# apple/ml-mdm

Measured on AMD Instinct MI355X. Metric: denoise-steps/sec, whole job = N x optimizer steps/s at per-GPU batch 64 (train fwd+bwd+optimizer, cc12m_64x64 U-Net), higher is better.
Workload: dtype bf16; 1 GPU; unet64 train step, per-GPU batch 64, global batch 64; global_batch=64, parallelism=dp1, settle_steps=15

## Files before the change

### ml-mdm_amd/csrc/gemm_conv.hip

```cpp
#include <stdio.h>
#include <stdlib.h>

#include <type_traits>
#include <utility>

#include "common.hpp"
#include "conv_args.hpp"

namespace mdm {



__device__ __forceinline__ void load4(const float* p, float (&o)[4]) {
  const f32x4 t = *reinterpret_cast<const f32x4*>(p);
  o[0] = t[0]; o[1] = t[1]; o[2] = t[2]; o[3] = t[3];
}
__device__ __forceinline__ void load4(const bf16* p, float (&o)[4]) {
  const bf16x4 t = *reinterpret_cast<const bf16x4*>(p);
  o[0] = (float)t[0]; o[1] = (float)t[1]; o[2] = (float)t[2]; o[3] = (float)t[3];
}

__device__ __attribute__((aligned(16))) uint4 g_zero_page[4] = {};


struct NoPrefetch { __device__ __forceinline__ void operator()() const {} };

template <typename T, int BM, int BN, int WM, int WN, int LDS_BYTES, typename AfterLds = NoPrefetch>
__device__ __forceinline__ void conv_epilogue(const ConvArgs& p, f32x4 (&acc)[BM / WM / 16][BN / WN / 16], char* smem,
                                              int m0, int n0, AfterLds after_lds = AfterLds()) {
  constexpr int EPV = Tr<T>::EPV;
  constexpr int NT_ = WM * WN * 64;
  constexpr int TM = BM / WM, TN = BN / WN;
  constexpr int MT = TM / 16, NT = TN / 16;
  const int tid = threadIdx.x, lane = tid & 63, wave = tid >> 6;
  const int wm = wave / WN, wn = wave % WN;
  const int quad = lane >> 4, l16 = lane & 15;
  T* __restrict__ Y = reinterpret_cast<T*>(p.y);
  T* __restrict__ Ypre = reinterpret_cast<T*>(p.ypre);
  const T* __restrict__ R = reinterpret_cast<const T*>(p.res);
  const T* __restrict__ AUX = reinterpret_cast<const T*>(p.aux);
  constexpr int OCH = BN / EPV;
  constexpr bool POW2 = (OCH & (OCH - 1)) == 0;
  constexpr int PITCH = BN * (int)sizeof(T) + (POW2 ? 0 : 16);
  constexpr int SWZ = POW2 ? (OCH >= 32 ? 32 : OCH) - 1 : 0;
  static_assert(BM * PITCH <= LDS_BYTES, "output tile must fit the k-loop LDS");
  if ((p.Cout % EPV) == 0) {
    f32x4 bv[NT];
#pragma unroll
    for (int j = 0; j < NT; ++j) {
      const int n = n0 + wn * TN + j * 16 + quad * 4;
      bv[j] = (p.bias && n < p.Cout) ? *reinterpret_cast<const f32x4*>(p.bias + n) : f32x4{0.f, 0.f, 0.f, 0.f};
    }
#pragma unroll
    for (int i = 0; i < MT; ++i) {
      const int ml = wm * TM + i * 16 + l16;
#pragma unroll
      for (int j = 0; j < NT; ++j) {
        const int nl = wn * TN + j * 16 + quad * 4;
        const f32x4 v = acc[i][j] + bv[j];
        constexpr int CPL = 16 / (4 * (int)sizeof(T));
        const int cl = nl / EPV;
        char* dst = smem + ml * PITCH + ((cl ^ (ml & SWZ)) << 4) + ((nl / 4) % CPL) * 8;
        if constexpr (sizeof(T) == 4) {
          *reinterpret_cast<f32x4*>(dst) = v;
        } else {
          *reinterpret_cast<bf16x4*>(dst) = bf16x4{(bf16)v[0], (bf16)v[1], (bf16)v[2], (bf16)v[3]};
        }
      }
    }
    constexpr int NCHP = BM * (BN / EPV) / NT_;
    constexpr bool AUX8 = sizeof(T) == 2 && kFfnAuxByte;
    const T* const PSRC = (p.act == 2 && AUX) ? AUX : R;
    uint4 pre[NCHP];
    if (AUX8 && p.act == 2 && AUX) {
      const unsigned char* const A8 = reinterpret_cast<const unsigned char*>(p.aux);
#pragma unroll
      for (int i = 0; i < NCHP; ++i) {
        const int idx = tid + i * NT_;
        const int row = idx / (BN / EPV), ch = idx - row * (BN / EPV);
        const int m = m0 + row, n = n0 + ch * EPV;
        pre[i] = uint4{0u, 0u, 0u, 0u};
        if (m < p.M && n < p.Cout) {
          const uint2 t = *reinterpret_cast<const uint2*>(A8 + (size_t)m * p.Cout + n);
          pre[i].x = t.x; pre[i].y = t.y;
        }
      }
    } else if (PSRC) {
#pragma unroll
      for (int i = 0; i < NCHP; ++i) {
        const int idx = tid + i * NT_;
        const int row = idx / (BN / EPV), ch = idx - row * (BN / EPV);
        const int m = m0 + row, n = n0 + ch * EPV;
        pre[i] = uint4{0u, 0u, 0u, 0u};
        if (m < p.M && n < p.Cout) {
          size_t o = (size_t)m * p.Cout + n;
          if (p.ps_cout > 0) {
            const int ph = n / p.ps_cout, co = n - ph * p.ps_cout;
            const int bw = m % p.ps_W, t_ = m / p.ps_W;
            const int bh = t_ % p.ps_H, img = t_ / p.ps_H;
            o = (((size_t)img * (2 * p.ps_H) + 2 * bh + (ph >> 1)) * (2 * p.ps_W) + 2 * bw + (ph & 1)) * p.ps_cout + co;
          }
          pre[i] = *reinterpret_cast<const uint4*>(PSRC + o);
        }
      }
    }
    __syncthreads();
    const int act = p.act;
    constexpr int NCH = BM * OCH / NT_;
    static_assert(NCH * NT_ == BM * OCH, "staged tile must divide evenly over the block");
    uint4 raw[NCH];
#pragma unroll
    for (int i = 0; i < NCH; ++i) {
      const int idx = tid + i * NT_;
      const int row = idx / OCH, ch = idx - row * OCH;
      raw[i] = *reinterpret_cast<const uint4*>(smem + row * PITCH + ((ch ^ (row & SWZ)) << 4));
    }
    __syncthreads();
    if (PSRC) __builtin_amdgcn_s_waitcnt(0x0F70);
    after_lds();
#pragma unroll
    for (int i = 0; i < NCH; ++i) {
      const int idx = tid + i * NT_;
      const int row = idx / OCH, ch = idx - row * OCH;
      const int m = m0 + row, n = n0 + ch * EPV;
      if (m >= p.M || n >= p.Cout) continue;
      size_t o = (size_t)m * p.Cout + n;
      if (p.ps_cout > 0) {
        const int ph = n / p.ps_cout, co = n - ph * p.ps_cout;
        const int bw = m % p.ps_W, t_ = m / p.ps_W;
        const int bh = t_ % p.ps_H, img = t_ / p.ps_H;
        o = (((size_t)img * (2 * p.ps_H) + 2 * bh + (ph >> 1)) * (2 * p.ps_W) + 2 * bw + (ph & 1)) * p.ps_cout + co;
      }
      if (act == 0 && !R) {
        *reinterpret_cast<uint4*>(Y + o) = raw[i];
        continue;
      }
      Chunk<T> c;
      c.load(reinterpret_cast<const T*>(&raw[i]));
      if (act == 1) {
        if (Ypre) {
          if constexpr (AUX8) {
            const uint2 code = {DGeluCode::enc4(&c.v[0]), DGeluCode::enc4(&c.v[4])};
            *reinterpret_cast<uint2*>(reinterpret_cast<unsigned char*>(p.ypre) + o) = code;
          } else {
            *reinterpret_cast<uint4*>(Ypre + o) = raw[i];
          }
        }
        gelu_vec<T, EPV>(c.v);
      } else if (act == 2) {
        if constexpr (AUX8) {
          float g[8];
          DGeluCode::dec4(pre[i].x, g);
          DGeluCode::dec4(pre[i].y, g + 4);
#pragma unroll
          for (int e = 0; e < EPV; ++e) c.v[e] *= g[e];
        } else {
          Chunk<T> ax;
          ax.load(reinterpret_cast<const T*>(&pre[i]));
          mul_dgelu_vec<T, EPV>(c.v, ax.v);
        }
      }
      if (R) {
        Chunk<T> rr;
        rr.load(reinterpret_cast<const T*>(&pre[i]));
#pragma unroll
        for (int e = 0; e < EPV; ++e) c.v[e] += rr.v[e];
      }
      c.store(Y + o);
    }
    return;
  }
  __syncthreads();
  after_lds();
#pragma unroll
  for (int i = 0; i < MT; ++i) {
    const int m = m0 + wm * TM + i * 16 + l16;
    if (m >= p.M) continue;
#pragma unroll
    for (int j = 0; j < NT; ++j) {
      const int n = n0 + wn * TN + j * 16 + quad * 4;
      if (n >= p.Cout) continue;
      float v[4] = {acc[i][j][0], acc[i][j][1], acc[i][j][2], acc[i][j][3]};
      const size_t o = (size_t)m * p.Cout + n;
      const int nv = min(4, p.Cout - n);
#pragma unroll
      for (int e = 0; e < 4; ++e) {
        if (e >= nv) continue;
        if (p.bias) v[e] += p.bias[n + e];
        if (p.act == 1) {
          if (Ypre) {
            if constexpr (sizeof(T) == 2 && kFfnAuxByte) reinterpret_cast<unsigned char*>(p.ypre)[o + e] = (unsigned char)DGeluCode::enc(to_f32(from_f32<T>(v[e])));
            else Ypre[o + e] = from_f32<T>(v[e]);
          }
          v[e] = gelu_t<T>(v[e]);
        } else if (p.act == 2) {
          if constexpr (sizeof(T) == 2 && kFfnAuxByte) v[e] *= DGeluCode::dec(reinterpret_cast<const unsigned char*>(p.aux)[o + e]);
          else v[e] *= dgelu_t<T>(to_f32(AUX[o + e]));
        }
        if (R) v[e] += to_f32(R[o + e]);
        Y[o + e] = from_f32<T>(v[e]);
      }
    }
  }
}

__device__ __forceinline__ void load_frag_planes(FragSplit& f, const char* t, int row, int quad) {
  f.hi = *reinterpret_cast<const bf16x8*>(t + lds_chunk_off(row, 2 * quad));
  f.lo = *reinterpret_cast<const bf16x8*>(t + lds_chunk_off(row, 2 * quad + 1));
}
template <typename F> __device__ __forceinline__ void load_frag_planes(F&, const char*, int, int) {}

template <typename T, int BM, int BN, int WM, int WN, int MODE, int SPLIT = 0>
__global__ __launch_bounds__(WM * WN * 64, 2) void conv_gemm_kernel(ConvArgs p) {
  constexpr int NSTAGE = 2;
  constexpr int EPV = Tr<T>::EPV, BK = Tr<T>::BK, KSTEPS = Tr<T>::KSTEPS;
  constexpr int NT_ = WM * WN * 64;
  constexpr int RPP = NT_ / 8;
  constexpr int TM = BM / WM, TN = BN / WN;
  constexpr int MT = TM / 16, NT = TN / 16;
  constexpr int AJ = BM / RPP, BJ = BN / RPP;
  constexpr int A_BYTES = BM * 128, B_BYTES = BN * 128, STAGE = A_BYTES + B_BYTES;
  static_assert(BM % RPP == 0 && BN % RPP == 0, "tile rows must be a multiple of the staging pass");
  extern __shared__ __attribute__((aligned(16))) char smem[];

  const int tid = threadIdx.x, lane = tid & 63, wave = tid >> 6;
  const int wm = wave / WN, wn = wave % WN;
  const int quad = lane >> 4, l16 = lane & 15;

  const int tiles_n = (p.Cout + BN - 1) / BN;
  const int t = xcd_remap(blockIdx.x, gridDim.x);
  const int m0 = (t / tiles_n) * BM, n0 = (t % tiles_n) * BN;

  const T* __restrict__ X = reinterpret_cast<const T*>(p.x);
  const T* __restrict__ Wp = reinterpret_cast<const T*>(p.w);

  const int lrow = tid >> 3;
  const int lchunk = (tid & 7) ^ (lrow & 7);
  int a_pix[AJ];
  int a_oh[AJ], a_ow[AJ];
#pragma unroll
  for (int j = 0; j < AJ; ++j) {
    const int m = m0 + lrow + RPP * j;
    if (m < p.M) {
      if (MODE == MODE_1x1) {
        a_pix[j] = m; a_oh[j] = 0; a_ow[j] = 0;
      } else {
        const int hw = p.Ho * p.Wo;
        const int n = m / hw, r = m - n * hw;
        const int oh = r / p.Wo;
        a_pix[j] = n * p.H * p.W; a_oh[j] = oh; a_ow[j] = r - oh * p.Wo;
      }
    } else {
      a_pix[j] = -1; a_oh[j] = 0; a_ow[j] = 0;
    }
  }
  int kcur = lchunk * EPV;
// ... 47 lines not shown

  f32x4 acc[MT][NT];
#pragma unroll
  for (int i = 0; i < MT; ++i)
#pragma unroll
    for (int j = 0; j < NT; ++j) acc[i][j] = f32x4{0.f, 0.f, 0.f, 0.f};

  const int ntiles = (p.K + BK - 1) / BK;
#define MDM_COMPUTE_TILE(cur)                                                                             \
  {                                                                                                       \
    const char* As = (cur);                                                                               \
    const char* Bs = (cur) + A_BYTES;                                                                     \
    _Pragma("unroll") for (int ks = 0; ks < KSTEPS; ++ks) {                                               \
      typename FragOf<T, SPLIT != 0>::type af[MT], bfr[NT];                                               \
      _Pragma("unroll") for (int i = 0; i < MT; ++i) load_frag_x(af[i], As, wm * TM + i * 16 + l16, ks, quad);    \
      _Pragma("unroll") for (int j = 0; j < NT; ++j) {                                                    \
        if constexpr (SPLIT == 2) load_frag_planes(bfr[j], Bs, wn * TN + j * 16 + l16, quad);             \
        else load_frag_x(bfr[j], Bs, wn * TN + j * 16 + l16, ks, quad);                                   \
      }                                                                                                   \
      _Pragma("unroll") for (int i = 0; i < MT; ++i)                                                      \
        _Pragma("unroll") for (int j = 0; j < NT; ++j) mma16(acc[i][j], bfr[j], af[i]);                   \
    }                                                                                                     \
  }
  MDM_STAGE_TILE(smem);
  __syncthreads();
  for (int kt = 0; kt < ntiles; ++kt) {
    char* cur = smem + (kt & 1) * STAGE;
    if (kt + 1 < ntiles) MDM_STAGE_TILE(smem + ((kt + 1) & 1) * STAGE);
    MDM_COMPUTE_TILE(cur);
    __syncthreads();
  }
#undef MDM_COMPUTE_TILE
#undef MDM_STAGE_TILE
#undef MDM_GLDS

  conv_epilogue<T, BM, BN, WM, WN, NSTAGE * STAGE>(p, acc, smem, m0, n0);
}

template <int NT, int DMA, int... I>
__device__ __forceinline__ void sched_rows(std::integer_sequence<int, I...>) {
  ((__builtin_amdgcn_sched_group_barrier(0x008, NT, I * 0), __builtin_amdgcn_sched_group_barrier(0x010, DMA, 0),
    __builtin_amdgcn_sched_group_barrier(0x100, 1, 0)), ...);
}

constexpr int CG_MAXG = 32;
struct ConvGroup {
  const void* x[CG_MAXG];
  const void* w[CG_MAXG];
  const float* bias[CG_MAXG];
  void* y[CG_MAXG];
};
struct NoConvGroup {};

template <int BM, int BN, int WM, int WN, int MODE, bool GROUPED = false, bool SPLITK = false, bool SEL4 = false, int NSTG = 2>
__global__ __launch_bounds__(WM * WN * 64, 2) void conv_gemm_bl_kernel(ConvArgs p, std::conditional_t<GROUPED, ConvGroup, NoConvGroup> gr) {
#if defined(__HIP_DEVICE_COMPILE__)
  using T = bf16;
  static_assert(!GROUPED || MODE == MODE_1x1, "grouped launches: 1x1 / linear only");
  static_assert(!(GROUPED && SPLITK), "split-K launches are single problems");
  static_assert(!SEL4 || (MODE == MODE_3x3 && !GROUPED && !SPLITK), "tap selection: plain 3x3 launches only");
  constexpr int NT_ = WM * WN * 64;
  constexpr int RPP = NT_ / 8;
  constexpr int TM = BM / WM, TN = BN / WN;
  constexpr int MT = TM / 16, NT = TN / 16;
  constexpr int AJ = BM / RPP, BJ = BN / RPP;
  constexpr int A_BYTES = BM * 128, B_BYTES = BN * 128, STAGE = A_BYTES + B_BYTES;
  constexpr unsigned INVALID = 0x7F000000u;
  static_assert(MODE == MODE_1x1 || MODE == MODE_3x3, "buffer-addressed loader: 1x1 and 3x3 only");
  static_assert(BM % RPP == 0 && BN % RPP == 0, "tile rows must be a multiple of the staging pass");
  extern __shared__ __attribute__((aligned(16))) char smem[];

  const int tid = threadIdx.x, lane = tid & 63, wave = tid >> 6;
  const int wm = wave / WN, wn = wave % WN;
  const int quad = lane >> 4, l16 = lane & 15;

  const int tiles_n = (p.Cout + BN - 1) / BN;
  const int tiles_per_problem = ((p.M + BM - 1) / BM) * tiles_n;
  const int tiles_total = tiles_per_problem * (GROUPED ? p.groups : 1) * (SPLITK ? p.ksplit : 1);
  const int G = gridDim.x;
  const int b_in_group = xcd_remap(blockIdx.x, G);

  const int lrow = tid >> 3;
  const int lchunk = (tid & 7) ^ (lrow & 7);
  const unsigned bias = MODE == MODE_3x3 ? (unsigned)(p.W + 1) * p.Cin * 2u : 0u;
  unsigned a_voff[AJ], a_mask[AJ], b_voff[BJ];
  int m0 = 0, n0 = 0, grp = 0;
  int sel_base_tile = p.sel_base;
  const int kpp_ = (p.sel_cout >> 6) * 4;
  int split = 0, kt0 = 0, nloc = p.K / 64;
  char* a_base = const_cast<char*>(reinterpret_cast<const char*>(p.x)) - bias;
  char* b_base = const_cast<char*>(reinterpret_cast<const char*>(p.w));
#define MDM_TILE_SETUP(tile_)                                                                               \
  {                                                                                                         \
    int tl_ = (tile_);                                                                                      \
    if constexpr (GROUPED) {                                                                                \
      grp = tl_ / tiles_per_problem; tl_ -= grp * tiles_per_problem;                                        \
      a_base = const_cast<char*>(reinterpret_cast<const char*>(gr.x[grp]));                                 \
      b_base = const_cast<char*>(reinterpret_cast<const char*>(gr.w[grp]));                                 \
    }                                                                                                       \
    if constexpr (SPLITK) {                                                                                 \
      split = tl_ / tiles_per_problem; tl_ -= split * tiles_per_problem;                                    \
      kt0 = split * p.kt_per; nloc = min(p.kt_per, p.K / 64 - kt0);                                         \
    }                                                                                                       \
    m0 = (tl_ / tiles_n) * BM; n0 = (tl_ % tiles_n) * BN;                                                   \
    if constexpr (SEL4) {                                                                                   \
      if (p.sel_mode == 1) { const int ph_ = n0 / p.sel_cout; sel_base_tile = (ph_ >> 1) * 3 + (ph_ & 1); } \
    }                                                                                                       \
    _Pragma("unroll") for (int j = 0; j < AJ; ++j) {                                                        \
      const int m = m0 + lrow + RPP * j;                                                                    \
      a_voff[j] = INVALID; a_mask[j] = 0u;                                                                  \
      if (m < p.M) {                                                                                        \
        if (MODE == MODE_1x1) {                                                                             \
          a_voff[j] = (unsigned)m * p.Cin * 2u + lchunk * 16u;                                              \
          a_mask[j] = 0x1ffu;                                                                               \
        } else {                                                                                            \
          const int hw = p.Ho * p.Wo;                                                                       \
          const int n = m / hw, r = m - n * hw;                                                             \
          const int oh = r / p.Wo, ow = r - oh * p.Wo;                                                      \
          const int ih0 = oh * p.stride, iw0 = ow * p.stride;                                               \
          a_voff[j] = (unsigned)(n * p.H * p.W + ih0 * p.W + iw0) * p.Cin * 2u + lchunk * 16u;              \
          unsigned mk = 0u;                                                                                 \
          _Pragma("unroll") for (int tp = 0; tp < 9; ++tp) {                                                \
            const int ih = ih0 + tp / 3 - 1, iw = iw0 + tp % 3 - 1;                                         \
            if ((unsigned)ih < (unsigned)p.H && (unsigned)iw < (unsigned)p.W) mk |= 1u << tp;               \
          }                                                                                                 \
          a_mask[j] = mk;                                                                                   \
        }                                                                                                   \
      }                                                                                                     \
    }                                                                                                       \
    _Pragma("unroll") for (int j = 0; j < BJ; ++j) {                                                        \
      const int n = n0 + lrow + RPP * j;                                                                    \
      b_voff[j] = n < p.Cout ? (unsigned)n * p.K * 2u + lchunk * 16u : INVALID;                             \
    }                                                                                                       \
    if (p.dev_flags & 2) {   \
      _Pragma("unroll") for (int j = 0; j < AJ; ++j) a_voff[j] = INVALID;                                   \
      _Pragma("unroll") for (int j = 0; j < BJ; ++j) b_voff[j] = INVALID;                                   \
    }                                                                                                       \
  }
  const unsigned a_bytes = (unsigned)p.N * p.H * p.W * p.Cin * 2u + bias;
  const unsigned b_bytes = (unsigned)p.Cout * p.K * 2u;
  const int wave_lds = __builtin_amdgcn_readfirstlane(wave * 1024);
  const int ntiles = p.K / 64;

#define MDM_BLDS(rs, lds_off, voff, soff)                                                                   \
  __builtin_amdgcn_raw_ptr_buffer_load_lds(rs, (__attribute__((address_space(3))) void*)(lds_off), 16, voff, soff, 0, 0)
#define MDM_TILE_STATE(kt_)                                                                                 \
  const bool more_ = (kt_) < (SPLITK ? nloc : ntiles);                                                      \
  const int kta_ = SPLITK ? kt0 + (kt_) : (kt_);                                                            \
  const auto rsA = __builtin_amdgcn_make_buffer_rsrc(a_base, 0, more_ ? a_bytes : 0u, 0x00020000);         \
  const auto rsB = __builtin_amdgcn_make_buffer_rsrc(b_base, 0, more_ ? b_bytes : 0u, 0x00020000);         \
  const int b_soff = kta_ * 128;                                                                            \
  int a_soff = b_soff, tapbit = 1;                                                                          \
  if (MODE == MODE_3x3) {                                                                                   \
    int cb, tap;                                                                                            \
    if constexpr (SEL4) {                                                                                   \
      int r_ = kta_, base_ = sel_base_tile, coff_ = 0;                                                      \
      if (p.sel_mode == 2) {                              \
        const int ph_ = (kta_ >= kpp_) + (kta_ >= 2 * kpp_) + (kta_ >= 3 * kpp_);                           \
        r_ = kta_ - ph_ * kpp_;                                                                             \
        base_ = (1 - (ph_ >> 1)) * 3 + (1 - (ph_ & 1));                                                     \
        coff_ = ph_ * (p.sel_cout >> 6);                                                                    \
      }                                                                                                     \
      cb = coff_ + (r_ >> 2);                                                                               \
      tap = base_ + (r_ & 1) + 3 * ((r_ >> 1) & 1);                                                         \
    } else {                                                                                                \
      cb = kta_ / 9; tap = kta_ - 9 * cb;                                                                   \
    }                                                                                                       \
    const int kh = (tap * 11) >> 5, kw = tap - 3 * kh;                                                      \
    a_soff = (kh * p.W + kw) * p.Cin * 2 + cb * 128;                                                        \
    tapbit = 1 << tap;                                                                                      \
  }
#define MDM_DMA_PIECE(stage, q)                                                                             \
  if ((q) < AJ) {                                                                                           \
    const unsigned vo = (MODE == MODE_1x1 || (a_mask[(q)] & tapbit)) ? a_voff[(q)] : INVALID;               \
    MDM_BLDS(rsA, (stage) + (q) * (RPP * 128) + wave_lds, vo, a_soff);                                      \
  } else if ((q) < AJ + BJ) {                                                                               \
    MDM_BLDS(rsB, (stage) + A_BYTES + ((q) - AJ) * (RPP * 128) + wave_lds, b_voff[(q) - AJ], b_soff);       \
  }

  f32x4 acc[MT][NT];

#define MDM_TILE_PROLOGUE()                                                                                 \
  {                                                                                                         \
    MDM_TILE_STATE(0);                                                                                      \
    _Pragma("unroll") for (int q = 0; q < AJ + BJ; ++q) { MDM_DMA_PIECE(smem, q); }                         \
  }                                                                                                         \
  {                                                                                                         \
    MDM_TILE_STATE(1);                                                                                      \
    _Pragma("unroll") for (int q = 0; q < AJ + BJ; ++q) { MDM_DMA_PIECE(smem + STAGE, q); }                 \
  }                                                                                                         \
  if constexpr (NSTG > 2) {                                                                                 \
    {                                                                                                       \
      MDM_TILE_STATE(2);                                                                                    \
      _Pragma("unroll") for (int q = 0; q < AJ + BJ; ++q) { MDM_DMA_PIECE(smem + 2 * STAGE, q); }           \
    }                                                                                                       \
    {                                                                                                       \
      MDM_TILE_STATE(3);                                                                                    \
      _Pragma("unroll") for (int q = 0; q < AJ + BJ; ++q) { MDM_DMA_PIECE(smem + 3 * STAGE, q); }           \
    }                                                                                                       \
  }

  int tile = b_in_group;
  if (tile >= tiles_total) return;
  MDM_TILE_SETUP(tile);
  MDM_TILE_PROLOGUE();
  for (;;) {
#pragma unroll
    for (int i = 0; i < MT; ++i)
#pragma unroll
      for (int j = 0; j < NT; ++j) acc[i][j] = f32x4{0.f, 0.f, 0.f, 0.f};
    asm volatile("s_waitcnt vmcnt(%0)" ::"n"((NSTG - 2) * (AJ + BJ) + (NSTG > 2 ? AJ + BJ : 0)) : "memory");
    __syncthreads();
    Frag<T> af[MT], b0[NT], b1[NT];
#pragma unroll
    for (int j = 0; j < NT; ++j) load_frag<T>(b0[j], smem + A_BYTES, wn * TN + j * 16 + l16, 0, quad);
#pragma unroll
    for (int i = 0; i < MT; ++i) load_frag<T>(af[i], smem, wm * TM + i * 16 + l16, 0, quad);
    constexpr int DMA_PER_ROW = (AJ + BJ + MT - 1) / MT;
    const int kt_end = SPLITK ? nloc : ntiles;
    for (int kt = 0; kt < kt_end; ++kt) {
      const char* As = smem + (kt % NSTG) * STAGE;
      const char* Bs = As + A_BYTES;
#pragma unroll
      for (int j = 0; j < NT; ++j) load_frag<T>(b1[j], Bs, wn * TN + j * 16 + l16, 1, quad);
#pragma unroll
      for (int i = 0; i < MT; ++i) {
#pragma unroll
        for (int j = 0; j < NT; ++j) mma16(acc[i][j], b0[j], af[i]);
        load_frag<T>(af[i], As, wm * TM + i * 16 + l16, 1, quad);
      }
      __builtin_amdgcn_sched_group_barrier(0x100, NT, 0);
      sched_rows<NT, 0>(std::make_integer_sequence<int, MT>{});
      __builtin_amdgcn_sched_barrier(0);
      asm volatile("s_waitcnt vmcnt(%0)" ::"n"((NSTG - 2) * (AJ + BJ)) : "memory");
      __syncthreads();
      __builtin_amdgcn_sched_barrier(0);
      const char* An = smem + ((kt + 1) % NSTG) * STAGE;
      const char* Bn = An + A_BYTES;
      char* dst = smem + (kt % NSTG) * STAGE;
      MDM_TILE_STATE(kt + NSTG);
#pragma unroll
      for (int j = 0; j < NT; ++j) load_frag<T>(b0[j], Bn, wn * TN + j * 16 + l16, 0, quad);
#pragma unroll
      for (int i = 0; i < MT; ++i) {
#pragma unroll
        for (int j = 0; j < NT; ++j) mma16(acc[i][j], b1[j], af[i]);
#pragma unroll
        for (int d = 0; d < DMA_PER_ROW; ++d) { MDM_DMA_PIECE(dst, i * DMA_PER_ROW + d); }
        load_frag<T>(af[i], An, wm * TM + i * 16 + l16, 0, quad);
      }
      __builtin_amdgcn_sched_group_barrier(0x100, NT, 0);
      sched_rows<NT, DMA_PER_ROW>(std::make_integer_sequence<int, MT>{});
      __builtin_amdgcn_sched_barrier(0);
    }
    asm volatile("s_waitcnt vmcnt(0)" ::: "memory");
    __syncthreads();
    const int cur_m0 = m0, cur_n0 = n0;
    const int next = tile + G;
    if constexpr (SPLITK) {
      float* __restrict__ P = p.part + (size_t)split * p.M * p.Cout;
      if (next < tiles_total) {
        MDM_TILE_SETUP(next);
        MDM_TILE_PROLOGUE();
      }
#pragma unroll
      for (int i = 0; i < MT; ++i) {
        const int m = cur_m0 + wm * TM + i * 16 + l16;
        if (m >= p.M) continue;
#pragma unroll
        for (int j = 0; j < NT; ++j) {
          const int n = cur_n0 + wn * TN + j * 16 + quad * 4;
          if (n < p.Cout) *reinterpret_cast<f32x4*>(P + (size_t)m * p.Cout + n) = acc[i][j];
        }
      }
    } else {
      ConvArgs pe = p;
      if constexpr (GROUPED) { pe.bias = gr.bias[grp]; pe.y = gr.y[grp]; }
      auto prefetch_next = [&]() {
        if (next < tiles_total) {
          MDM_TILE_SETUP(next);
          MDM_TILE_PROLOGUE();
        }
      };
      conv_epilogue<T, BM, BN, WM, WN, NSTG * STAGE, decltype(prefetch_next)>(pe, acc, smem, cur_m0, cur_n0, prefetch_next);
    }
    if (next >= tiles_total) break;
    tile = next;
  }
#undef MDM_TILE_PROLOGUE
#undef MDM_TILE_SETUP
#undef MDM_DMA_PIECE
#undef MDM_TILE_STATE
#undef MDM_BLDS
#endif
}

struct WgradArgs {
  const void* x;
  const void* dy;
  float* slab;
  float* bslab;
  int N, H, W, Cin, Ho, Wo, Cout, stride;
  int M, K;
  int splits, mtiles_per_split;
  int groups;
  int bias_share;
  int skip_cout;
};

constexpr int WG_MAXG = 32;
constexpr int WG_BHDR = 64;
constexpr int WG_BSHARE = 4;
struct WgradGroup {
  const void* x[WG_MAXG];
  const void* dy[WG_MAXG];
  float* out[WG_MAXG];
  float* bout[WG_MAXG];
};

template <typename T, int MODE>
__global__ __launch_bounds__(256) void conv_wgrad_kernel(WgradArgs p) {
  constexpr int EPV = Tr<T>::EPV, BKM = Tr<T>::BK, KSTEPS = Tr<T>::KSTEPS;
  constexpr int BM = 128, BN = 128;
  constexpr int TM = 64, TN = 64, MT = 4, NT = 4;
  constexpr int A_BYTES = BM * 128, STAGE = 2 * A_BYTES;
  constexpr int CPR = 128 / EPV;
  constexpr int MB = BKM / EPV;
  constexpr int BLOCKS = CPR * MB;
  constexpr int NB = 2 * BLOCKS / 256;
  extern __shared__ __attribute__((aligned(16))) char smem[];

  const int tid = threadIdx.x, lane = tid & 63, wave = tid >> 6;
  const int wm = wave >> 1, wn = wave & 1;
  const int quad = lane >> 4, l16 = lane & 15;

  const int tiles_k = (p.K + BN - 1) / BN;
  const int tiles_n = (p.Cout + BM - 1) / BM;
  const int tiles = tiles_k * tiles_n;
  const int lid = xcd_remap(blockIdx.x, gridDim.x);
  const int split = lid / tiles;
  const int t = lid - split * tiles;
  const int n0 = (t / tiles_k) * BM, k0 = (t % tiles_k) * BN;

  const T* __restrict__ X = reinterpret_cast<const T*>(p.x);
  const T* __restrict__ DY = reinterpret_cast<const T*>(p.dy);

  int b_op[NB], b_cc[NB], b_mb[NB];
  int b_tap[NB], b_cin[NB];
// ... 1113 lines not shown
    t[co_l][r] = w[((size_t)(co0 + co_l) * Cin + ci0) * 9 + r];
  }
  __syncthreads();
  for (int e = tid; e < 4 * 16 * 256; e += 256) {
    const int co_l = e & 63, j = (e >> 6) & 3, ci_l = (e >> 8) & 15, phase = e >> 12;
    const int ph = phase >> 1, pw = phase & 1, dh = j >> 1, dw = j & 1;
    const int kh = ph == 0 ? (dh == 0 ? 1 : -1) : (dh == 0 ? 2 : 0);
    const int kw = pw == 0 ? (dw == 0 ? 1 : -1) : (dw == 0 ? 2 : 0);
    const float v = (kh >= 0 && kw >= 0) ? t[co_l][ci_l * 9 + kh * 3 + kw] : 0.f;
    w_sel[(((size_t)(phase * Cin + ci0 + ci_l) * (Cout >> 6) + (co0 >> 6)) * 4 + j) * 64 + co_l] = (bf16)v;
  }
}

__global__ __launch_bounds__(256) void upconv_wfold_kernel(const float* __restrict__ dwb, float* __restrict__ dw, int Cout,
                                                           int Cin, int accumulate) {
  const int idx = blockIdx.x * 256 + threadIdx.x;
  if (idx >= Cout * Cin) return;
  const int co = idx / Cin, ci = idx - co * Cin;
  float o[9];
#pragma unroll
  for (int k = 0; k < 9; ++k) o[k] = 0.f;
#pragma unroll
  for (int ph = 0; ph < 2; ++ph)
#pragma unroll
    for (int pw = 0; pw < 2; ++pw)
#pragma unroll
      for (int a = 0; a < 2; ++a)
#pragma unroll
        for (int b = 0; b < 2; ++b) {
          const float g = dwb[((size_t)((ph * 2 + pw) * Cout + co) * Cin + ci) * 9 + (ph + a) * 3 + (pw + b)];
#pragma unroll
          for (int kh = 0; kh < 3; ++kh)
#pragma unroll
            for (int kw = 0; kw < 3; ++kw)
              if (up_tap_in(ph, a, kh) && up_tap_in(pw, b, kw)) o[kh * 3 + kw] += g;
        }
#pragma unroll
  for (int k = 0; k < 9; ++k) {
    float* d = dw + (size_t)idx * 9 + k;
    *d = accumulate ? *d + o[k] : o[k];
  }
}

__global__ __launch_bounds__(256) void upconv_bfold_kernel(const float* __restrict__ db4, float* __restrict__ db, int Cout,
                                                           int accumulate) {
  const int co = blockIdx.x * 256 + threadIdx.x;
  if (co >= Cout) return;
  const float v = (db4[co] + db4[Cout + co]) + (db4[2 * Cout + co] + db4[3 * Cout + co]);
  db[co] = accumulate ? db[co] + v : v;
}

static int g_dev_flags = 0;
static inline ConvArgs with_dev_flags(const ConvArgs& a) { ConvArgs b = a; b.dev_flags = g_dev_flags; return b; }
static thread_local char g_last_gemm[96] = "";
extern "C" const char* mdm_last_gemm_kernel(void) { return g_last_gemm; }
#define MDM_NOTE_KERNEL(...) snprintf(g_last_gemm, sizeof(g_last_gemm), __VA_ARGS__)
template <typename T, int BM, int BN, int WM, int WN, int MODE, int SPLIT = 0>
static int launch_conv_cfg(const ConvArgs& a_, hipStream_t st) {
  const ConvArgs a = with_dev_flags(a_);
  constexpr int smem = 2 * (BM + BN) * 128;
  auto kern = conv_gemm_kernel<T, BM, BN, WM, WN, MODE, SPLIT>;
  ensure_dynamic_lds(kern, smem);
  const int tiles = ((a.M + BM - 1) / BM) * ((a.Cout + BN - 1) / BN);
  hipLaunchKernelGGL(kern, dim3(tiles), dim3(WM * WN * 64), smem, st, a);
  MDM_NOTE_KERNEL("conv_gemm_kernel<%s, %d, %d, %d, %d, %d>", sizeof(T) == 2 ? "bf16" : (SPLIT == 2 ? "float (bf16x3, weight planes)" : (SPLIT ? "float (bf16x3)" : "float")), BM, BN, WM, WN, MODE);
  MDM_LAUNCH_STATUS();
}

template <int BM, int BN, int WM, int WN, int MODE>
static int launch_conv_bl(const ConvArgs& a_, hipStream_t st) {
  const ConvArgs a = with_dev_flags(a_);
  constexpr int smem = 2 * (BM + BN) * 128;
  auto kern = conv_gemm_bl_kernel<BM, BN, WM, WN, MODE>;
  ensure_dynamic_lds(kern, smem);
  const int tiles = ((a.M + BM - 1) / BM) * ((a.Cout + BN - 1) / BN);
  if constexpr (BM == 128 && BN == 128) {
    if (tiles <= device_cus()) {
      auto kern4 = conv_gemm_bl_kernel<BM, BN, WM, WN, MODE, false, false, false, 4>;
      ensure_dynamic_lds(kern4, 2 * smem);
      hipLaunchKernelGGL(kern4, dim3(tiles), dim3(WM * WN * 64), 2 * smem, st, a, NoConvGroup{});
      MDM_NOTE_KERNEL("conv_gemm_bl_kernel<%d, %d, %d, %d, %d, 4 stages>", BM, BN, WM, WN, MODE);
      MDM_LAUNCH_STATUS();
    }
  }
  const int resident = device_cus() * (WM * WN == 4 ? 2 : 1);
  hipLaunchKernelGGL(kern, dim3(tiles < resident ? tiles : resident), dim3(WM * WN * 64), smem, st, a, NoConvGroup{});
  MDM_NOTE_KERNEL("conv_gemm_bl_kernel<%d, %d, %d, %d, %d>", BM, BN, WM, WN, MODE);
  MDM_LAUNCH_STATUS();
}

template <int BM, int BN, int WM, int WN>
static int launch_conv_bl_sel4(const ConvArgs& a_, hipStream_t st) {
  const ConvArgs a = with_dev_flags(a_);
  constexpr int smem = 2 * (BM + BN) * 128;
  auto kern = conv_gemm_bl_kernel<BM, BN, WM, WN, MODE_3x3, false, false, true>;
  ensure_dynamic_lds(kern, smem);
  const int tiles = ((a.M + BM - 1) / BM) * ((a.Cout + BN - 1) / BN);
  const int resident = device_cus() * (WM * WN == 4 ? 2 : 1);
  hipLaunchKernelGGL(kern, dim3(tiles < resident ? tiles : resident), dim3(WM * WN * 64), smem, st, a, NoConvGroup{});
  MDM_NOTE_KERNEL("conv_gemm_bl_kernel<%d, %d, %d, %d, %d, sel4>", BM, BN, WM, WN, MODE_3x3);
  MDM_LAUNCH_STATUS();
}

template <int BM, int BN, int WM, int WN>
static int launch_conv_bl_grouped(const ConvArgs& a_, const ConvGroup& gr, hipStream_t st) {
  const ConvArgs a = with_dev_flags(a_);
  constexpr int smem = 2 * (BM + BN) * 128;
  auto kern = conv_gemm_bl_kernel<BM, BN, WM, WN, MODE_1x1, true>;
  ensure_dynamic_lds(kern, smem);
  const int tiles = ((a.M + BM - 1) / BM) * ((a.Cout + BN - 1) / BN) * a.groups;
  const int resident = device_cus() * (WM * WN == 4 ? 2 : 1);
  hipLaunchKernelGGL(kern, dim3(tiles < resident ? tiles : resident), dim3(WM * WN * 64), smem, st, a, gr);
  MDM_NOTE_KERNEL("conv_gemm_bl_kernel<%d, %d, %d, %d, %d, grouped>", BM, BN, WM, WN, MODE_1x1);
  MDM_LAUNCH_STATUS();
}

template <typename T, int MODE>
static bool conv_bl_ok(const ConvArgs& a) {
  if (sizeof(T) != 2 || MODE == MODE_3x3_T2) return false;
  if (a.K % 64 != 0 || (MODE == MODE_3x3 && a.kblk == 0)) return false;
  const size_t lim = 0x7F000000u;
  const size_t bias = MODE == MODE_3x3 ? (size_t)(a.W + 1) * a.Cin * 2 : 0;
  if ((size_t)a.N * a.H * a.W * a.Cin * 2 + bias > lim || (size_t)a.Cout * a.K * 2 > lim) return false;
  return 2 * bias + (size_t)a.K * 2 < 0x00F00000u;
}

static int conv_ksplit(int M, int Cout, int K, int dtype) {
  if (dtype != DT_BF16 || K % 64 != 0 || Cout % 8 != 0 || Cout <= 64) return 1;
  constexpr int fill = 80, minkt = 6, minsave = 16;
  const long tiles = (long)((M + 127) / 128) * ((Cout + 127) / 128);
  const int nt = K / 64, cus = device_cus();
  if (tiles * 100 > (long)fill * 2 * cus || nt < 2 * minkt) return 1;
  const int per_cu = M <= 2048 ? 1 : 2;
  long sp = ((long)per_cu * cus) / tiles;
  if (sp > nt / minkt) sp = nt / minkt;
  if (sp > 16) sp = 16;
  if (sp < 2 || nt - (nt + sp - 1) / sp < minsave) return 1;
  return (int)sp;
}

extern "C" int mdm_conv_fwd_plan(int M, int Cout, int K, int dtype, int* splits, size_t* ws_bytes) {
  MDM_CHECK_ARG(splits && ws_bytes && M > 0 && Cout > 0 && K > 0);
  *splits = conv_ksplit(M, Cout, K, dtype);
  *ws_bytes = *splits > 1 ? (size_t)*splits * M * Cout * sizeof(float) : 0;
  return 0;
}

template <int MODE>
static int launch_conv_bl_splitk(ConvArgs a, int splits, float* ws, hipStream_t st) {
  a.dev_flags = g_dev_flags;
  constexpr int BM = 128, BN = 128, WM = 2, WN = 2;
  constexpr int smem = 2 * (BM + BN) * 128;
  auto kern = conv_gemm_bl_kernel<BM, BN, WM, WN, MODE, false, true>;
  ensure_dynamic_lds(kern, smem);
  const int nt = a.K / 64;
  a.kt_per = (nt + splits - 1) / splits;
  a.ksplit = (nt + a.kt_per - 1) / a.kt_per;
  a.part = ws;
  const int tiles = ((a.M + BM - 1) / BM) * ((a.Cout + BN - 1) / BN) * a.ksplit;
  const int resident = device_cus() * 2;
  if (tiles <= device_cus()) {
    auto kern4 = conv_gemm_bl_kernel<BM, BN, WM, WN, MODE, false, true, false, 4>;
    ensure_dynamic_lds(kern4, 2 * smem);
    hipLaunchKernelGGL(kern4, dim3(tiles), dim3(WM * WN * 64), 2 * smem, st, a, NoConvGroup{});
  } else
// ... 323 lines not shown
                               int Cout, int dtype, void* stream) {
  MDM_CHECK_ARG(x && w_ph && y && dtype == DT_BF16);
  MDM_CHECK_ARG(N > 0 && H > 0 && W > 0 && Cin % 64 == 0 && Cout > 0);
  const int tile = sel4_tile(Cout);
  MDM_CHECK_ARG(tile != 0);
  ConvArgs a = {};
  a.x = x; a.w = w_ph; a.bias = bias4; a.y = y;
  a.N = N; a.H = H; a.W = W; a.Cin = Cin; a.Ho = H; a.Wo = W; a.Cout = 4 * Cout; a.stride = 1;
  a.M = N * H * W; a.K = 4 * Cin; a.kblk = 64; a.ksplit = 1;
  a.sel_mode = 1; a.sel_cout = Cout;
  a.ps_cout = Cout; a.ps_H = H; a.ps_W = W;
  MDM_CHECK_ARG((conv_bl_ok<bf16, MODE_3x3>(a)));
  return launch_sel4(a, tile, reinterpret_cast<hipStream_t>(stream));
}

extern "C" int mdm_conv_up_dgrad(const void* dyb, const void* w_t, void* dx, int N, int H, int W, int Cout, int Cin,
                                 int dtype, void* stream) {
  MDM_CHECK_ARG(dyb && w_t && dx && dtype == DT_BF16);
  MDM_CHECK_ARG(N > 0 && H > 0 && W > 0 && Cout % 64 == 0 && Cin % 8 == 0);
  ConvArgs a = {};
  a.x = dyb; a.w = w_t; a.y = dx;
  a.N = N; a.H = H; a.W = W; a.Cin = 4 * Cout; a.Ho = H; a.Wo = W; a.Cout = Cin; a.stride = 1;
  a.M = N * H * W; a.K = 16 * Cout; a.kblk = 64; a.ksplit = 1;
  a.sel_mode = 2; a.sel_cout = Cout;
  MDM_CHECK_ARG((conv_bl_ok<bf16, MODE_3x3>(a)));
  const int code = conv_tile_code(a.M, a.Cout, DT_BF16);
  return launch_sel4(a, code == 256256 ? 256 : (code == 256192 ? 192 : 128), reinterpret_cast<hipStream_t>(stream));
}

extern "C" int mdm_linear_grouped(const void* const* x, const void* const* w_packed, const float* const* bias,
                                  void* const* y, int groups, int M, int Cin, int Cout, int dtype, void* stream) {
  MDM_CHECK_ARG(x && w_packed && y && groups >= 1 && groups <= CG_MAXG);
  MDM_CHECK_ARG(dtype == DT_BF16 && Cin % 64 == 0 && Cout % 8 == 0 && M > 0);
  ConvArgs a = {};
  a.N = M; a.H = 1; a.W = 1; a.Cin = Cin; a.Ho = 1; a.Wo = 1; a.Cout = Cout; a.stride = 1;
  a.M = M; a.K = Cin; a.act = 0; a.kblk = 0; a.groups = groups;
  MDM_CHECK_ARG((size_t)M * Cin * 2 <= 0x7F000000u && (size_t)Cout * Cin * 2 <= 0x7F000000u);
  ConvGroup gr = {};
  for (int g = 0; g < groups; ++g) {
    MDM_CHECK_ARG(x[g] && w_packed[g] && y[g]);
    gr.x[g] = x[g]; gr.w[g] = w_packed[g]; gr.bias[g] = bias ? bias[g] : nullptr; gr.y[g] = y[g];
  }
  a.x = gr.x[0]; a.w = gr.w[0]; a.y = gr.y[0];
  hipStream_t st = reinterpret_cast<hipStream_t>(stream);
  const int code = conv_tile_code(M * groups, Cout, DT_BF16);
  if (code == 256256) return launch_conv_bl_grouped<256, 256, 2, 4>(a, gr, st);
  if (code == 256192) return launch_conv_bl_grouped<256, 192, 2, 4>(a, gr, st);
  return launch_conv_bl_grouped<128, 128, 2, 2>(a, gr, st);
}

extern "C" int mdm_dev_ffn_aux_bytes(void) { return kFfnAuxByte ? 1 : 2; }

extern "C" int mdm_dev_set_knob(int idx, int value) {
  MDM_CHECK_ARG(idx == 0 || idx == 2 || idx == 8);
  if (idx == 0) g_dev_flags = value ? 2 : 0;
  else if (idx == 2) g_force_tile = value;
  else g_no_wgrad_direct = value;
  return 0;
}

struct WgDirectArgs {
  const bf16* x; const bf16* dy; float* slab; float* bslab;
  int N, H, W, tiles_x, tiles_y, tiles;
};
constexpr int wgd_pitch(int bytes) {
  int d = bytes / 4;
  while (d % 64 != 20 && d % 64 != 52) ++d;
  return d * 4;
}
typedef __attribute__((ext_vector_type(4))) short wg_s16x4;
__device__ __forceinline__ Frag<bf16> wgd_tr2(const char* p, int second) {
  const wg_s16x4 a = __builtin_amdgcn_ds_read_tr16_b64_v4i16((__attribute__((address_space(3))) wg_s16x4*)(p));
  const wg_s16x4 b = __builtin_amdgcn_ds_read_tr16_b64_v4i16((__attribute__((address_space(3))) wg_s16x4*)(p + second));
  typedef __attribute__((ext_vector_type(8))) short s16x8;
  s16x8 v = {a[0], a[1], a[2], a[3], b[0], b[1], b[2], b[3]};
  Frag<bf16> f;
  f.v = __builtin_bit_cast(bf16x8, v);
  return f;
}

template <int CIN, int TAPS, int TH>
__global__ __launch_bounds__(512, 1) void wgrad_direct_kernel(WgDirectArgs p) {
  constexpr int COUT = 64, TW = 32, HALO = TAPS == 9 ? 1 : 0;
  constexpr int TWH = TW + 2 * HALO, THH = TH + 2 * HALO;
  constexpr int XCH = CIN / 8, DCH = COUT / 8;
  constexpr int PX = wgd_pitch(CIN * 2), PD = wgd_pitch(COUT * 2);
  constexpr int K = TAPS * CIN;
  constexpr int NBW = K / 16 / 4;
  static_assert((K / 16) % 4 == 0, "K columns split over 4 waves");
  constexpr int XROW = TWH * XCH, XCHUNKS = THH * XROW, DCHUNKS = TH * TW * DCH;
  constexpr int NXL = (XCHUNKS + 511) / 512, NDL = (DCHUNKS + 511) / 512;
  extern __shared__ __attribute__((aligned(16))) char dsm[];
  char* const xs = dsm;
  char* const ys = dsm + THH * TWH * PX;
  const int tid = threadIdx.x, lane = tid & 63, wid = tid >> 6;
  const int l15 = lane & 15, quad = lane >> 4;
  const int mw = wid >> 2, nw = wid & 3;

  const int trow = 8 * quad + (l15 >> 2), tseg = (l15 & 3) * 8;
  int y_off[2], x_off[NBW];
#pragma unroll
  for (int mi = 0; mi < 2; ++mi) y_off[mi] = trow * PD + (mw * 2 + mi) * 32 + tseg;
#pragma unroll
  for (int nb = 0; nb < NBW; ++nb) {
    const int nbg = nw * NBW + nb, tap = nbg / (CIN / 16), cb = nbg - tap * (CIN / 16);
    const int dy_ = TAPS == 9 ? tap / 3 : 0, dx_ = TAPS == 9 ? tap % 3 : 0;
    x_off[nb] = (dy_ * TWH + dx_ + trow) * PX + cb * 32 + tseg;
  }

// ... 399 lines not shown
```

Before: 11.51 steps/s.

## Use counted vmcnt waits to overlap epilogue stores with next-tile prefetch

In the persistent conv GEMM kernel, the first k-tile is peeled and its vmcnt wait now counts how many global stores the previous tile's epilogue issued. That lets the next tile's prologue loads complete without draining those outstanding stores. The prologue DMA is emitted as inline asm so the compiler cannot insert conservative waits, and the epilogue now reports its store count. A grid-cap knob is also added, which is off by default. The change risks correctness if the store count is wrong, and it now always waits on the LDS counter in the epilogue.

```diff
diff --git a/ml-mdm_amd/csrc/gemm_conv.hip b/ml-mdm_amd/csrc/gemm_conv.hip
--- a/ml-mdm_amd/csrc/gemm_conv.hip
+++ b/ml-mdm_amd/csrc/gemm_conv.hip
@@ -25,14 +25,22 @@
 
 struct NoPrefetch { __device__ __forceinline__ void operator()() const {} };
 
+enum { EPI_STORES_UNKNOWN = 0, EPI_STORES_1 = 1, EPI_STORES_2 = 2 };
+template <typename T, int BM, int BN, int NT_> constexpr int conv_epilogue_nch = BM * (BN / Tr<T>::EPV) / NT_;
+
 template <typename T, int BM, int BN, int WM, int WN, int LDS_BYTES, typename AfterLds = NoPrefetch>
-__device__ __forceinline__ void conv_epilogue(const ConvArgs& p, f32x4 (&acc)[BM / WM / 16][BN / WN / 16], char* smem,
-                                              int m0, int n0, AfterLds after_lds = AfterLds()) {
+__device__ __forceinline__ int conv_epilogue(const ConvArgs& p, f32x4 (&acc)[BM / WM / 16][BN / WN / 16], char* smem,
+                                             int m0, int n0, AfterLds after_lds = AfterLds()) {
   constexpr int EPV = Tr<T>::EPV;
   constexpr int NT_ = WM * WN * 64;
   constexpr int TM = BM / WM, TN = BN / WN;
   constexpr int MT = TM / 16, NT = TN / 16;
-  const int tid = threadIdx.x, lane = tid & 63, wave = tid >> 6;
+  int tid = threadIdx.x;
+  if constexpr (!std::is_same_v<AfterLds, NoPrefetch>) {
+    asm volatile("" : "+v"(tid));
+    tid &= NT_ - 1;
+  }
+  const int lane = tid & 63, wave = tid >> 6;
   const int wm = wave / WN, wn = wave % WN;
   const int quad = lane >> 4, l16 = lane & 15;
   T* __restrict__ Y = reinterpret_cast<T*>(p.y);
@@ -106,7 +114,8 @@
     }
     __syncthreads();
     const int act = p.act;
-    constexpr int NCH = BM * OCH / NT_;
+    constexpr int NCH = conv_epilogue_nch<T, BM, BN, NT_>;
+    const int kind = (m0 + BM <= p.M && n0 + BN <= p.Cout) ? ((act == 1 && Ypre) ? EPI_STORES_2 : EPI_STORES_1) : EPI_STORES_UNKNOWN;
     static_assert(NCH * NT_ == BM * OCH, "staged tile must divide evenly over the block");
     uint4 raw[NCH];
 #pragma unroll
@@ -116,7 +125,7 @@
       raw[i] = *reinterpret_cast<const uint4*>(smem + row * PITCH + ((ch ^ (row & SWZ)) << 4));
     }
     __syncthreads();
-    if (PSRC) __builtin_amdgcn_s_waitcnt(0x0F70);
+    __builtin_amdgcn_s_waitcnt(0x0F70);
     after_lds();
 #pragma unroll
     for (int i = 0; i < NCH; ++i) {
@@ -168,7 +177,7 @@
       }
       c.store(Y + o);
     }
-    return;
+    return kind;
   }
   __syncthreads();
   after_lds();
@@ -202,6 +211,7 @@
       }
     }
   }
+  return EPI_STORES_UNKNOWN;
 }
 
 __device__ __forceinline__ void load_frag_planes(FragSplit& f, const char* t, int row, int quad) {
@@ -355,6 +365,8 @@
 };
 struct NoConvGroup {};
 
+#pragma clang diagnostic push
+#pragma clang diagnostic ignored "-Winline-asm"
 template <int BM, int BN, int WM, int WN, int MODE, bool GROUPED = false, bool SPLITK = false, bool SEL4 = false, int NSTG = 2>
 __global__ __launch_bounds__(WM * WN * 64, 2) void conv_gemm_bl_kernel(ConvArgs p, std::conditional_t<GROUPED, ConvGroup, NoConvGroup> gr) {
 #if defined(__HIP_DEVICE_COMPILE__)
@@ -447,6 +459,11 @@
 
 #define MDM_BLDS(rs, lds_off, voff, soff)                                                                   \
   __builtin_amdgcn_raw_ptr_buffer_load_lds(rs, (__attribute__((address_space(3))) void*)(lds_off), 16, voff, soff, 0, 0)
+  typedef int mdm_rsrc_words __attribute__((ext_vector_type(4)));
+#define MDM_BLDS_TEXT(rs, lds_off, voff, soff)                                                              \
+  asm volatile("s_mov_b32 m0, %0\n\tbuffer_load_dwordx4 %1, %2, %3 offen lds"                               \
+               ::"s"((unsigned)(__UINTPTR_TYPE__)(__attribute__((address_space(3))) char*)(lds_off)), "v"(voff), "s"(rs), "s"(soff) \
+               : "memory", "m0")
 #define MDM_TILE_STATE(kt_)                                                                                 \
   const bool more_ = (kt_) < (SPLITK ? nloc : ntiles);                                                      \
   const int kta_ = SPLITK ? kt0 + (kt_) : (kt_);                                                            \
@@ -480,17 +497,40 @@
   } else if ((q) < AJ + BJ) {                                                                               \
     MDM_BLDS(rsB, (stage) + A_BYTES + ((q) - AJ) * (RPP * 128) + wave_lds, b_voff[(q) - AJ], b_soff);       \
   }
+#define MDM_TILE_STATE_TEXT(kt_)                                                                            \
+  MDM_TILE_STATE(kt_)                                                                                       \
+  const unsigned long long ab_ = (unsigned long long)a_base, bb_ = (unsigned long long)b_base;              \
+  const mdm_rsrc_words twA = {(int)(unsigned)ab_, (int)((unsigned)(ab_ >> 32) & 0xffffu), (int)(more_ ? a_bytes : 0u), 0x00020000}; \
+  const mdm_rsrc_words twB = {(int)(unsigned)bb_, (int)((unsigned)(bb_ >> 32) & 0xffffu), (int)(more_ ? b_bytes : 0u), 0x00020000};
+#define MDM_DMA_PIECE_TEXT(stage, q)                                                                        \
+  if ((q) < AJ) {                                                                                           \
+    const unsigned vo = (MODE == MODE_1x1 || (a_mask[(q)] & tapbit)) ? a_voff[(q)] : INVALID;               \
+    MDM_BLDS_TEXT(twA, (stage) + (q) * (RPP * 128) + wave_lds, vo, a_soff);                                 \
+  } else if ((q) < AJ + BJ) {                                                                               \
+    MDM_BLDS_TEXT(twB, (stage) + A_BYTES + ((q) - AJ) * (RPP * 128) + wave_lds, b_voff[(q) - AJ], b_soff);  \
+  }
 
   f32x4 acc[MT][NT];
 
 #define MDM_TILE_PROLOGUE()                                                                                 \
-  {                                                                                                         \
-    MDM_TILE_STATE(0);                                                                                      \
-    _Pragma("unroll") for (int q = 0; q < AJ + BJ; ++q) { MDM_DMA_PIECE(smem, q); }                         \
-  }                                                                                                         \
-  {                                                                                                         \
-    MDM_TILE_STATE(1);                                                                                      \
-    _Pragma("unroll") for (int q = 0; q < AJ + BJ; ++q) { MDM_DMA_PIECE(smem + STAGE, q); }                 \
+  if constexpr (NSTG == 2 && !SPLITK) {               \
+    {                                                                                                       \
+      MDM_TILE_STATE_TEXT(0);                                                                               \
+      _Pragma("unroll") for (int q = 0; q < AJ + BJ; ++q) { MDM_DMA_PIECE_TEXT(smem, q); }                  \
+    }                                                                                                       \
+    {                                                                                                       \
+      MDM_TILE_STATE_TEXT(1);                                                                               \
+      _Pragma("unroll") for (int q = 0; q < AJ + BJ; ++q) { MDM_DMA_PIECE_TEXT(smem + STAGE, q); }          \
+    }                                                                                                       \
+  } else {                                                                                                  \
+    {                                                                                                       \
+      MDM_TILE_STATE(0);                                                                                    \
+      _Pragma("unroll") for (int q = 0; q < AJ + BJ; ++q) { MDM_DMA_PIECE(smem, q); }                       \
+    }                                                                                                       \
+    {                                                                                                       \
+      MDM_TILE_STATE(1);                                                                                    \
+      _Pragma("unroll") for (int q = 0; q < AJ + BJ; ++q) { MDM_DMA_PIECE(smem + STAGE, q); }               \
+    }                                                                                                       \
   }                                                                                                         \
   if constexpr (NSTG > 2) {                                                                                 \
     {                                                                                                       \
@@ -503,6 +543,49 @@
     }                                                                                                       \
   }
 
+#define MDM_K_TILE(kt, MID_WAIT)                                                                            \
+  {                                                                                                         \
+    const char* As = smem + ((kt) % NSTG) * STAGE;                                                          \
+    const char* Bs = As + A_BYTES;                                                                          \
+                                                                                          \
+    _Pragma("unroll") for (int j = 0; j < NT; ++j) load_frag<T>(b1[j], Bs, wn * TN + j * 16 + l16, 1, quad); \
+    _Pragma("unroll") for (int i = 0; i < MT; ++i) {                                                        \
+      _Pragma("unroll") for (int j = 0; j < NT; ++j) mma16(acc[i][j], b0[j], af[i]);                        \
+      load_frag<T>(af[i], As, wm * TM + i * 16 + l16, 1, quad);                                             \
+    }                                                                                                       \
+    __builtin_amdgcn_sched_group_barrier(0x100, NT, 0);                                                     \
+    sched_rows<NT, 0>(std::make_integer_sequence<int, MT>{});                                               \
+    __builtin_amdgcn_sched_barrier(0);                                                                      \
+    MID_WAIT();                                                                                             \
+    __syncthreads();                                                                                        \
+    __builtin_amdgcn_sched_barrier(0);                                                                      \
+                                                                                          \
+    const char* An = smem + (((kt) + 1) % NSTG) * STAGE;                                                    \
+    const char* Bn = An + A_BYTES;                                                                          \
+    char* dst = smem + ((kt) % NSTG) * STAGE;                                                               \
+    MDM_TILE_STATE((kt) + NSTG);                                                                            \
+    _Pragma("unroll") for (int j = 0; j < NT; ++j) load_frag<T>(b0[j], Bn, wn * TN + j * 16 + l16, 0, quad); \
+    _Pragma("unroll") for (int i = 0; i < MT; ++i) {                                                        \
+      _Pragma("unroll") for (int j = 0; j < NT; ++j) mma16(acc[i][j], b1[j], af[i]);                        \
+      _Pragma("unroll") for (int d = 0; d < DMA_PER_ROW; ++d) { MDM_DMA_PIECE(dst, i * DMA_PER_ROW + d); }  \
+      load_frag<T>(af[i], An, wm * TM + i * 16 + l16, 0, quad);                                             \
+    }                                                                                                       \
+    __builtin_amdgcn_sched_group_barrier(0x100, NT, 0);                                                     \
+    sched_rows<NT, DMA_PER_ROW>(std::make_integer_sequence<int, MT>{});                                     \
+    __builtin_amdgcn_sched_barrier(0);                                                                      \
+  }
+#define MDM_WAIT_STEADY() asm volatile("s_waitcnt vmcnt(%0)" ::"n"((NSTG - 2) * (AJ + BJ)) : "memory")
+#define MDM_WAIT_COUNTED(P_)                                                                                \
+  if (prev_stores == EPI_STORES_UNKNOWN) asm volatile("s_waitcnt vmcnt(%0)" ::"n"(P_) : "memory");          \
+  else if (prev_stores == EPI_STORES_1) asm volatile("s_waitcnt vmcnt(%0)" ::"n"(NCH + (P_)) : "memory");   \
+  else asm volatile("s_waitcnt vmcnt(%0)" ::"n"(2 * NCH + (P_)) : "memory")
+#define MDM_WAIT_HEAD_MID() MDM_WAIT_COUNTED(0)
+
+  constexpr bool PEEL = NSTG == 2 && !SPLITK;
+  constexpr int NCH = conv_epilogue_nch<T, BM, BN, NT_>;
+  static_assert(2 * NCH + 2 * (AJ + BJ) <= 63, "counted waits: 6-bit vmcnt");
+  int prev_stores = EPI_STORES_UNKNOWN;
+
   int tile = b_in_group;
   if (tile >= tiles_total) return;
   MDM_TILE_SETUP(tile);
@@ -512,7 +595,11 @@
     for (int i = 0; i < MT; ++i)
 #pragma unroll
       for (int j = 0; j < NT; ++j) acc[i][j] = f32x4{0.f, 0.f, 0.f, 0.f};
-    asm volatile("s_waitcnt vmcnt(%0)" ::"n"((NSTG - 2) * (AJ + BJ) + (NSTG > 2 ? AJ + BJ : 0)) : "memory");
+    if constexpr (PEEL) {
+      MDM_WAIT_COUNTED(AJ + BJ);
+    } else {
+      asm volatile("s_waitcnt vmcnt(%0)" ::"n"((NSTG - 2) * (AJ + BJ) + (NSTG > 2 ? AJ + BJ : 0)) : "memory");
+    }
     __syncthreads();
     Frag<T> af[MT], b0[NT], b1[NT];
 #pragma unroll
@@ -521,41 +608,8 @@
     for (int i = 0; i < MT; ++i) load_frag<T>(af[i], smem, wm * TM + i * 16 + l16, 0, quad);
     constexpr int DMA_PER_ROW = (AJ + BJ + MT - 1) / MT;
     const int kt_end = SPLITK ? nloc : ntiles;
-    for (int kt = 0; kt < kt_end; ++kt) {
-      const char* As = smem + (kt % NSTG) * STAGE;
-      const char* Bs = As + A_BYTES;
-#pragma unroll
-      for (int j = 0; j < NT; ++j) load_frag<T>(b1[j], Bs, wn * TN + j * 16 + l16, 1, quad);
-#pragma unroll
-      for (int i = 0; i < MT; ++i) {
-#pragma unroll
-        for (int j = 0; j < NT; ++j) mma16(acc[i][j], b0[j], af[i]);
-        load_frag<T>(af[i], As, wm * TM + i * 16 + l16, 1, quad);
-      }
-      __builtin_amdgcn_sched_group_barrier(0x100, NT, 0);
-      sched_rows<NT, 0>(std::make_integer_sequence<int, MT>{});
-      __builtin_amdgcn_sched_barrier(0);
-      asm volatile("s_waitcnt vmcnt(%0)" ::"n"((NSTG - 2) * (AJ + BJ)) : "memory");
-      __syncthreads();
-      __builtin_amdgcn_sched_barrier(0);
-      const char* An = smem + ((kt + 1) % NSTG) * STAGE;
-      const char* Bn = An + A_BYTES;
-      char* dst = smem + (kt % NSTG) * STAGE;
-      MDM_TILE_STATE(kt + NSTG);
-#pragma unroll
-      for (int j = 0; j < NT; ++j) load_frag<T>(b0[j], Bn, wn * TN + j * 16 + l16, 0, quad);
-#pragma unroll
-      for (int i = 0; i < MT; ++i) {
-#pragma unroll
-        for (int j = 0; j < NT; ++j) mma16(acc[i][j], b1[j], af[i]);
-#pragma unroll
-        for (int d = 0; d < DMA_PER_ROW; ++d) { MDM_DMA_PIECE(dst, i * DMA_PER_ROW + d); }
-        load_frag<T>(af[i], An, wm * TM + i * 16 + l16, 0, quad);
-      }
-      __builtin_amdgcn_sched_group_barrier(0x100, NT, 0);
-      sched_rows<NT, DMA_PER_ROW>(std::make_integer_sequence<int, MT>{});
-      __builtin_amdgcn_sched_barrier(0);
-    }
+    if constexpr (PEEL) MDM_K_TILE(0, MDM_WAIT_HEAD_MID);
+    for (int kt = PEEL ? 1 : 0; kt < kt_end; ++kt) MDM_K_TILE(kt, MDM_WAIT_STEADY);
     asm volatile("s_waitcnt vmcnt(0)" ::: "memory");
     __syncthreads();
     const int cur_m0 = m0, cur_n0 = n0;
@@ -585,18 +639,26 @@
           MDM_TILE_PROLOGUE();
         }
       };
-      conv_epilogue<T, BM, BN, WM, WN, NSTG * STAGE, decltype(prefetch_next)>(pe, acc, smem, cur_m0, cur_n0, prefetch_next);
+      prev_stores = conv_epilogue<T, BM, BN, WM, WN, NSTG * STAGE, decltype(prefetch_next)>(pe, acc, smem, cur_m0, cur_n0, prefetch_next);
     }
     if (next >= tiles_total) break;
     tile = next;
   }
+#undef MDM_WAIT_HEAD_MID
+#undef MDM_WAIT_COUNTED
+#undef MDM_WAIT_STEADY
+#undef MDM_K_TILE
 #undef MDM_TILE_PROLOGUE
 #undef MDM_TILE_SETUP
+#undef MDM_DMA_PIECE_TEXT
+#undef MDM_TILE_STATE_TEXT
+#undef MDM_BLDS_TEXT
 #undef MDM_DMA_PIECE
 #undef MDM_TILE_STATE
 #undef MDM_BLDS
 #endif
 }
+#pragma clang diagnostic pop
 
 struct WgradArgs {
   const void* x;
@@ -1816,6 +1878,11 @@
 
 static int g_dev_flags = 0;
 static inline ConvArgs with_dev_flags(const ConvArgs& a) { ConvArgs b = a; b.dev_flags = g_dev_flags; return b; }
+static int g_grid_cap = 0;
+static inline int persistent_grid(int tiles, int resident) {
+  const int g = tiles < resident ? tiles : resident;
+  return g_grid_cap > 0 && g > g_grid_cap ? g_grid_cap : g;
+}
 static thread_local char g_last_gemm[96] = "";
 extern "C" const char* mdm_last_gemm_kernel(void) { return g_last_gemm; }
 #define MDM_NOTE_KERNEL(...) snprintf(g_last_gemm, sizeof(g_last_gemm), __VA_ARGS__)
@@ -1839,7 +1906,7 @@
   ensure_dynamic_lds(kern, smem);
   const int tiles = ((a.M + BM - 1) / BM) * ((a.Cout + BN - 1) / BN);
   if constexpr (BM == 128 && BN == 128) {
-    if (tiles <= device_cus()) {
+    if (tiles <= persistent_grid(tiles, device_cus())) {
       auto kern4 = conv_gemm_bl_kernel<BM, BN, WM, WN, MODE, false, false, false, 4>;
       ensure_dynamic_lds(kern4, 2 * smem);
       hipLaunchKernelGGL(kern4, dim3(tiles), dim3(WM * WN * 64), 2 * smem, st, a, NoConvGroup{});
@@ -1848,7 +1915,7 @@
     }
   }
   const int resident = device_cus() * (WM * WN == 4 ? 2 : 1);
-  hipLaunchKernelGGL(kern, dim3(tiles < resident ? tiles : resident), dim3(WM * WN * 64), smem, st, a, NoConvGroup{});
+  hipLaunchKernelGGL(kern, dim3(persistent_grid(tiles, resident)), dim3(WM * WN * 64), smem, st, a, NoConvGroup{});
   MDM_NOTE_KERNEL("conv_gemm_bl_kernel<%d, %d, %d, %d, %d>", BM, BN, WM, WN, MODE);
   MDM_LAUNCH_STATUS();
 }
@@ -1861,7 +1928,7 @@
   ensure_dynamic_lds(kern, smem);
   const int tiles = ((a.M + BM - 1) / BM) * ((a.Cout + BN - 1) / BN);
   const int resident = device_cus() * (WM * WN == 4 ? 2 : 1);
-  hipLaunchKernelGGL(kern, dim3(tiles < resident ? tiles : resident), dim3(WM * WN * 64), smem, st, a, NoConvGroup{});
+  hipLaunchKernelGGL(kern, dim3(persistent_grid(tiles, resident)), dim3(WM * WN * 64), smem, st, a, NoConvGroup{});
   MDM_NOTE_KERNEL("conv_gemm_bl_kernel<%d, %d, %d, %d, %d, sel4>", BM, BN, WM, WN, MODE_3x3);
   MDM_LAUNCH_STATUS();
 }
@@ -1874,7 +1941,7 @@
   ensure_dynamic_lds(kern, smem);
   const int tiles = ((a.M + BM - 1) / BM) * ((a.Cout + BN - 1) / BN) * a.groups;
   const int resident = device_cus() * (WM * WN == 4 ? 2 : 1);
-  hipLaunchKernelGGL(kern, dim3(tiles < resident ? tiles : resident), dim3(WM * WN * 64), smem, st, a, gr);
+  hipLaunchKernelGGL(kern, dim3(persistent_grid(tiles, resident)), dim3(WM * WN * 64), smem, st, a, gr);
   MDM_NOTE_KERNEL("conv_gemm_bl_kernel<%d, %d, %d, %d, %d, grouped>", BM, BN, WM, WN, MODE_1x1);
   MDM_LAUNCH_STATUS();
 }
@@ -2304,9 +2371,10 @@
 extern "C" int mdm_dev_ffn_aux_bytes(void) { return kFfnAuxByte ? 1 : 2; }
 
 extern "C" int mdm_dev_set_knob(int idx, int value) {
-  MDM_CHECK_ARG(idx == 0 || idx == 2 || idx == 8);
+  MDM_CHECK_ARG(idx == 0 || idx == 2 || idx == 3 || idx == 8);
   if (idx == 0) g_dev_flags = value ? 2 : 0;
   else if (idx == 2) g_force_tile = value;
+  else if (idx == 3) g_grid_cap = value > 0 ? value : 0;
   else g_no_wgrad_direct = value;
   return 0;
 }
```

Result: no change. 11.54 steps/s, median of 2 (+0.3%).
